# widkyyu/Goal-conditioned-Reinforcement-Learning-with-environmental-and-policy-priors

Measured on AMD Instinct MI355X. Metric: env-steps/sec, higher is better.
Workload: dtype u8

## Files before the change

goal-conditioned-reinforcement-learning-with-environmental-and-policy-priors_amd/_lib.py:

```python
import ctypes as C
import os
import subprocess

_PKG_DIR = os.path.dirname(os.path.abspath(__file__))
LIB_PATH = os.path.join(_PKG_DIR, "libtwoarmy_hip.so")
CSRC_DIR = os.path.join(_PKG_DIR, "csrc")

TW_CELLS = 289
TW_REC_WORDS = 48
TW_DRAW_WORDS = 8
TW_F_AUTORESET = 1
TW_F_POLICY_IDX = 2
TW_F_MATRIX_CODE = 4
TW_F_SLAB_HIPMALLOC = 8

FIELDS = dict(AX=0, AY=1, DIR=2, STEP_COUNT=3, STEP_MOVE=4, PONE=5, PATROL=6, UP1=7, RIGHT2=8, UPD_LONG=9,
              UPD_HORIZ=10, RISK=11, FIRST_ROOM2=12, OBX=13, OBY=16, O1X=19, O1Y=22, O1_VALID=25, O2X=26,
              O2Y=30, O2_VALID=34, GOAL_X=35, GOAL_Y=36, T=37, ERROR=38, MAX_STEPS=39, EPISODES=40,
              LAST_REWARD=41, LAST_TERM=42, LAST_TRUNC=43, WALL_I1=44, WALL_I2=45)

LAUNCH_FIELDS = ("pipelined", "PG", "LAYOUT", "pipe_grid", "E", "FAST", "seq_grid", "T")

ENV_ERRORS = {1: AttributeError, 2: AssertionError, 3: TypeError}

# ... 105 lines not shown
    "mg_nav_path_scan": (C.c_int, [_vp, _i64, _i, _i, _i, _i, _vp, _vp, _vp, _vp, _vp, _vp, _i, _vp, _vp, _vp, _vp, _vp, _vp,
                                   _vp, _vp, _vp]),
    "mg_nav_path_summary_workspace": (C.c_int, [_i, _i]),
    "mg_nav_path_summary": (C.c_int, [_vp, _vp, _vp, _vp, _vp, _vp, _i, _i, _vp, _vp, _vp]),
    "ppo_her_relabel": (C.c_int, [_vp, _vp, _vp, _vp, _vp, _vp, _u64, C.c_uint32, C.c_uint32, _i, _i, _i, _vp, _vp, _vp,
                                  _vp, _vp, _vp, _vp, _vp]),
    "ppo_her_relabel_window": (C.c_int, [_vp, _vp, _vp, _vp, _vp, _vp, _u64, C.c_uint32, C.c_uint32, _i, _i, _i, _i, _vp,
                                         _vp, _vp, _vp, _vp, _vp, _vp, _vp]),
    "ppo_lstm_cell": (C.c_int, [_vp, _vp, C.c_longlong, _vp, _vp, _vp, _i, _i, _vp]),
    "ppo_decoder_frames": (C.c_int, [_vp, _i, _vp, _vp, _vp, _vp, _vp, C.c_float, _vp, _vp]),
    "ppo_gather_stack_u8": (C.c_int, [_vp, _i, _vp, _i, _vp, _vp, _vp, _vp, _vp, _i, _vp, _vp, _vp]),
    "ppo_age_scan": (C.c_int, [_vp, _vp, _vp, _i, _i, _vp, _vp]),
    "ppo_episode_scan": (C.c_int, [_vp, _vp, _vp, _i, _i, _vp, _vp, _vp, _vp, _vp]),
    "ppo_episode_summary": (C.c_int, [_vp, _vp, _vp, _vp, _vp, _vp, _i, _i, _i, C.c_double, C.c_double, _vp, _vp, _vp, _vp,
                                      _vp, _vp]),
    "ppo_episode_summary_workspace": (C.c_int, [_i, _i]),
    "ppo_visit_scan": (C.c_int, [_vp, _vp, _vp, _i, _i, _i, _i, _vp, _vp, _vp, _vp]),
    "ppo_visit_carry_words": (C.c_int, [_i, _i, _i]),
    "ppo_visit_hist": (C.c_int, [_vp, _i, _i, _vp, _vp, _vp, _i, _i, _i, _vp, _vp]),
    "ppo_bonus_table_words": (C.c_int, [_i, _i, _i, _i, _i, _i]),
    "ppo_bonus_workspace_bytes": (_i64, [_i, _i, _i, _i, _i, _i]),
    "ppo_bonus_scan": (C.c_int, [_vp, _vp, _vp, C.c_long, C.c_long, _vp, _vp, _i, _i, _i, _i, _i, _i, _i, C.c_double, _vp, _vp,
                                 _vp, _vp, _vp, _vp, _vp]),
    "ppo_bonus_episode_words": (C.c_int, [_i, _i, _i, _i, _i]),
    "ppo_bonus_scan_episode": (C.c_int, [_vp, _vp, _vp, C.c_long, C.c_long, _vp, _vp, _vp, _vp, _i, _i, _i, _i, _i, _i, _i,
                                         C.c_double, _vp, _vp, _vp, _vp, _vp, _vp]),
    "ppo_bias_relu_nhwc": (C.c_int, [_vp, _vp, _i64, _i, _vp]),
    "ppo_conv1_up4_bias_relu": (C.c_int, [_vp, _i, _i, _vp, _vp, _vp, _vp]),
    "ppo_conv1_up4_bias_relu_c": (C.c_int, [_vp, _i, _i, _i, _vp, _vp, _vp, _vp]),
    "ppo_conv1_up4_bwd_groups": (C.c_int, [_i]),
    "ppo_conv1_up4_bwd": (C.c_int, [_vp, _i, _i, _vp, _vp, _vp, _vp, _vp]),
    "ppo_relu_bwd_bias_grad_nhwc_blocks": (C.c_int, [_i64, _i]),
    "ppo_relu_bwd_bias_grad_nhwc": (C.c_int, [_vp, _vp, _vp, _vp, _i64, _i, _vp]),
})

_lib = None


def exported_symbols():
    return sorted(_SIGS)


def lib():
    global _lib
    if _lib is None:
        if not os.path.exists(LIB_PATH):
            raise TwoarmyLibraryError(
                "%s not built: run `python -c 'import __graft_entry__ as g; g.build()'` "
                "(hipcc --offload-arch=gfx950); there is no CPU fallback" % LIB_PATH)
        import torch
        try:
            h = C.CDLL(LIB_PATH)
        except OSError as ex:
            raise TwoarmyLibraryError("cannot load %s: %s" % (LIB_PATH, ex)) from ex
        for name, (res, args) in _SIGS.items():
            try:
                fn = getattr(h, name)
            except AttributeError as ex:
                raise TwoarmyLibraryError("%s lacks symbol %s" % (LIB_PATH, name)) from ex
            fn.restype, fn.argtypes = res, args
        runtimes = set()
        try:
            with open("/proc/self/maps") as f:
                for line in f:
                    if "libamdhip64" in line:
                        runtimes.add(line.split()[-1])
# ... 17 lines not shown
```

goal-conditioned-reinforcement-learning-with-environmental-and-policy-priors_amd/csrc/ppo_kernels.hip:

```cpp

#include <hip/hip_runtime.h>
#include <float.h>
#include <stdint.h>

#include <type_traits>

#include "launch.h"
#include "philox.h"
#include "twoarmy.h"
#include "twoarmy_ppo.h"

namespace {

constexpr float CAT_EPS = FLT_EPSILON;

template <int A> __device__ __forceinline__ float cat_row(const float *__restrict__ row, float (&p)[A]) {
    float S = 0.f;
#pragma unroll
    for (int k = 0; k < A; ++k) { p[k] = row[k]; S += p[k]; }
    return S;
}
__device__ __forceinline__ float cat_log(float q) { return logf(fminf(fmaxf(q, CAT_EPS), 1.0f - CAT_EPS)); }

template <typename T, int K> __device__ __forceinline__ void block_sum(T (&v)[K], T *lds) {
    const int tid = threadIdx.x;
#pragma unroll
    for (int k = 0; k < K; ++k) lds[k * 256 + tid] = v[k];
    __syncthreads();
    for (int s = 128; s > 0; s >>= 1) {
        if (tid < s) {
#pragma unroll
            for (int k = 0; k < K; ++k) lds[k * 256 + tid] += lds[k * 256 + tid + s];
        }
        __syncthreads();
    }
#pragma unroll
    for (int k = 0; k < K; ++k) v[k] = lds[k * 256];
}

__device__ __forceinline__ float4 relu4(float4 v) {
    return make_float4(fmaxf(v.x, 0.f), fmaxf(v.y, 0.f), fmaxf(v.z, 0.f), fmaxf(v.w, 0.f));
}
__device__ __forceinline__ float4 mask4(float4 g, float4 y) {
    return make_float4(y.x > 0.f ? g.x : 0.f, y.y > 0.f ? g.y : 0.f, y.z > 0.f ? g.z : 0.f, y.w > 0.f ? g.w : 0.f);
}
__device__ __forceinline__ void add4(float4 &acc, const float4 &o) { acc.x += o.x; acc.y += o.y; acc.z += o.z; acc.w += o.w; }
__device__ __forceinline__ float4 fma4(float x, float4 w, float4 acc) {
    return make_float4(fmaf(x, w.x, acc.x), fmaf(x, w.y, acc.y), fmaf(x, w.z, acc.z), fmaf(x, w.w, acc.w));
}

__device__ __forceinline__ float4 slot_sum4(const float4 *red, int rows, int stride, int cq) {
    float4 sum = red[cq];
    for (int r = 1; r < rows; ++r) add4(sum, red[r * stride + cq]);
    return sum;
}

__device__ __forceinline__ uint32_t done_at(const uint8_t *__restrict__ terminated, const uint8_t *__restrict__ truncated,
                                            size_t i) {
    return (uint32_t)(terminated[i] | truncated[i]);
}

template <int A>
__global__ void ppo_sample_kernel(const float *__restrict__ probs, int B, const float *__restrict__ uniforms,
                                  uint32_t k0, uint32_t k1, uint64_t offset, const uint64_t *__restrict__ offset_dev,
                                  int32_t *__restrict__ action, float *__restrict__ logp) {
    const int b = blockIdx.x * blockDim.x + threadIdx.x;
    if (b >= B) return;
    float p[A];
    const float sum = cat_row<A>(probs + (size_t)b * A, p);
    float u;
    if (uniforms) u = uniforms[b];
    else {
        const uint64_t ctr = (uint64_t)b + offset + (offset_dev ? *offset_dev : 0ull);
        uint32_t c0 = (uint32_t)ctr, c1 = (uint32_t)(ctr >> 32), c2 = 0, c3 = 0x54574F53u;
        philox4x32_10(k0, k1, c0, c1, c2, c3);
        u = (float)(c0 >> 8) * (1.0f / 16777216.0f);
    }
    int a = A - 1, last = A - 1;
    float cum = 0.f, qa = 0.f;
    bool found = false;
#pragma unroll
    for (int k = 0; k < A; ++k) {
        const float q = p[k] / sum;
        cum += q;
        if (q > 0.f) last = k;
        if (!found && cum > u) { a = k; found = true; }
    }
    if (!found) a = last;
#pragma unroll
    for (int k = 0; k < A; ++k) if (k == a) qa = p[k] / sum;
    action[b] = a;
    logp[b] = cat_log(qa);
}

__global__ __launch_bounds__(256) void ppo_bias_relu_kernel(float4 *__restrict__ y, const float4 *__restrict__ bias,
                                                            size_t n4, int c4) {
    const size_t stride = (size_t)gridDim.x * blockDim.x;
    for (size_t i = (size_t)blockIdx.x * blockDim.x + threadIdx.x; i < n4; i += stride) {
        float4 v = y[i];
        add4(v, bias[i % c4]);
        y[i] = relu4(v);
    }
}

__global__ __launch_bounds__(256) void ppo_relu_bwd_bias_grad_kernel(const float4 *__restrict__ gy,
                                                                     const float4 *__restrict__ y,
                                                                     float4 *__restrict__ gx,
                                                                     float4 *__restrict__ partial, size_t n_pixels,
                                                                     int c4, int pixels_per_block) {
    __shared__ float4 red[256];
    const int rows = 256 / c4;
    const int cq = threadIdx.x % c4, row = threadIdx.x / c4;
    const size_t p0 = (size_t)blockIdx.x * pixels_per_block;
    const size_t p1 = p0 + pixels_per_block < n_pixels ? p0 + pixels_per_block : n_pixels;
    float4 acc = make_float4(0.f, 0.f, 0.f, 0.f);
    if (row < rows) {
        for (size_t px = p0 + row; px < p1; px += rows) {
            const size_t i = px * c4 + cq;
            const float4 o = mask4(gy[i], y[i]);
            gx[i] = o;
            add4(acc, o);
        }
    }
    red[threadIdx.x] = acc;
    __syncthreads();
    if (row == 0) partial[(size_t)blockIdx.x * c4 + cq] = slot_sum4(red, rows, c4, cq);
}

template <int F> __device__ __forceinline__ void conv1_stage_frame(float *xs, const float *__restrict__ src, int tid) {
    for (int i = tid; i < F * 324; i += 256) {
        const int c = i / 324, r = i - c * 324, y = r / 18, x = r - y * 18;
        xs[i] = (y < 17 && x < 17) ? src[c * 289 + y * 17 + x] : 0.f;
    }
}

template <int F, int CQ>
__global__ __launch_bounds__(256) void ppo_conv1_up4_kernel(const float *__restrict__ frames, const float4 *__restrict__ wf,
                                                            const float4 *__restrict__ bias, float4 *__restrict__ out, int B) {
    __shared__ float xs[F * 18 * 18];
    constexpr int SLOTS = 256 / CQ;
    const int b = blockIdx.x, tid = threadIdx.x;
    const int cq = tid % CQ, slot = tid / CQ;
    conv1_stage_frame<F>(xs, frames + (size_t)b * F * 289, tid);
    __syncthreads();
    const float4 bv = bias[cq];
    float4 *dst = out + (size_t)b * 1089 * CQ;
#pragma unroll 1
    for (int ph = 0; ph < 4; ++ph) {
        const int py = ph >> 1, px = ph & 1;
        float4 w[4 * F];
#pragma unroll
        for (int k = 0; k < 4 * F; ++k) w[k] = wf[(ph * 4 * F + k) * CQ + cq];
        const int ny = 17 - py, nx = 17 - px;
        for (int q = slot; q < ny * nx; q += SLOTS) {
            const int m = q / nx, n = q - m * nx;
            float4 acc = bv;
#pragma unroll
            for (int t = 0; t < 4; ++t) {
                const int ty = t >> 1, tx = t & 1;
#pragma unroll
                for (int c = 0; c < F; ++c) acc = fma4(xs[c * 324 + (m + ty) * 18 + n + tx], w[t * F + c], acc);
            }
            dst[((2 * m + py) * 33 + 2 * n + px) * CQ + cq] = relu4(acc);
        }
    }
}

template <int F>
__global__ __launch_bounds__(256) void ppo_conv1_up4_bwd_kernel(const float *__restrict__ frames, const float4 *__restrict__ gy,
                                                                const float4 *__restrict__ y, float4 *__restrict__ gw_part,
                                                                float4 *__restrict__ gb_part, int B) {
    __shared__ float xs[F * 18 * 18];
    __shared__ float4 red[256];
    const int tid = threadIdx.x, cq = tid & 15, slot = tid >> 4;
    const int ph = blockIdx.y, py = ph >> 1, px = ph & 1;
    const int ny = 17 - py, nx = 17 - px;
    float4 acc[4 * F];
#pragma unroll
    for (int k = 0; k < 4 * F; ++k) acc[k] = make_float4(0.f, 0.f, 0.f, 0.f);
    float4 accb = make_float4(0.f, 0.f, 0.f, 0.f);
    for (int b = blockIdx.x; b < B; b += gridDim.x) {
        __syncthreads();
        conv1_stage_frame<F>(xs, frames + (size_t)b * F * 289, tid);
        __syncthreads();
        const size_t base = (size_t)b * 1089 * 16;
        for (int q = slot; q < ny * nx; q += 16) {
            const int m = q / nx, n = q - m * nx;
            const size_t o = base + (size_t)((2 * m + py) * 33 + 2 * n + px) * 16 + cq;
            const float4 g = mask4(gy[o], y[o]);
            add4(accb, g);
#pragma unroll
            for (int t = 0; t < 4; ++t) {
                const int ty = t >> 1, tx = t & 1;
#pragma unroll
                for (int c = 0; c < F; ++c) acc[t * F + c] = fma4(xs[c * 324 + (m + ty) * 18 + n + tx], g, acc[t * F + c]);
            }
        }
    }
    const size_t wbase = ((size_t)blockIdx.x * 4 + ph) * (4 * F) * 16;
#pragma unroll
    for (int k = 0; k <= 4 * F; ++k) {
        __syncthreads();
        red[tid] = k < 4 * F ? acc[k < 4 * F ? k : 0] : accb;
        __syncthreads();
        if (slot == 0) {
            const float4 sum = slot_sum4(red, 16, 16, cq);
            if (k < 4 * F) gw_part[wbase + (size_t)k * 16 + cq] = sum;
            else gb_part[((size_t)blockIdx.x * 4 + ph) * 16 + cq] = sum;
        }
    }
}

constexpr int GT = 64;

template <int GN>
__global__ __launch_bounds__(256) void ppo_gae_kernel(const float *__restrict__ reward, const float *__restrict__ value,
                                                      const float *__restrict__ next_value,
                                                      const uint8_t *__restrict__ done, float gamma, float lambda,
                                                      int use_done_mask, int T, int N, float *__restrict__ adv,
                                                      float *__restrict__ target, float *__restrict__ ret) {
    __shared__ float sd[GT][GN + 1];
    __shared__ float sc[GT][GN + 1];
// ... 924 lines not shown
int blocks(int64_t n, int per) { return (int)((n + per - 1) / per); }
int blocks_capped(int64_t n, int per, int cap) { return (int)((n + per - 1) / per < cap ? (n + per - 1) / per : cap); }
int ep_summary_blocks(int64_t M) { return blocks_capped(M, EP_BLOCK_ELEMS, EP_MAX_BLOCKS); }
float4 *f4(float *p) { return reinterpret_cast<float4 *>(p); }
const float4 *f4(const float *p) { return reinterpret_cast<const float4 *>(p); }
template <int V> using int_c = std::integral_constant<int, V>;

#define PPO_ACTION_COUNTS(X) X(5) X(2) X(3) X(4) X(7)
bool ppo_actions_ok(int A) {
#define PPO_IS(V) if (A == V) return true;
    PPO_ACTION_COUNTS(PPO_IS)
#undef PPO_IS
    return false;
}
template <typename Fn> void ppo_with_actions(int A, Fn &&fn) {
    switch (A) {
#define PPO_CASE(V) case V: fn(int_c<V>{}); break;
    PPO_ACTION_COUNTS(PPO_CASE)
#undef PPO_CASE
    }
}

template <typename FT>
int gather_stack(const char *what, const FT *frames, int frame_pitch, const float *pos_frames, int N, const int32_t *k_idx,
                 const int32_t *n_idx, const int32_t *age, const float *init_frame, const float *init_pos, int B,
                 float *out, float *pos_out, void *stream) {
    if (!all_set(frames, k_idx, n_idx, age, init_frame, out) || B <= 0 || frame_pitch < TW_CELLS) return TW_E_ARG;
    if (pos_out && !all_set(pos_frames, init_pos)) return TW_E_ARG;
    hipLaunchKernelGGL(ppo_gather_stack_kernel<FT>, dim3(blocks(B, 4)), dim3(256), 0, (hipStream_t)stream, frames, frame_pitch,
                       pos_frames, N, k_idx, n_idx, age, init_frame, init_pos, B, out, pos_out);
    return tw_launched(what);
}

}

extern "C" {

int ppo_sample(const float *probs, int B, int A, const float *uniforms, uint64_t seed, uint64_t offset,
               int32_t *action, float *logp, void *stream) {
    return ppo_sample_dev(probs, B, A, uniforms, seed, offset, nullptr, action, logp, stream);
}

int ppo_sample_dev(const float *probs, int B, int A, const float *uniforms, uint64_t seed, uint64_t offset,
                   const uint64_t *offset_dev, int32_t *action, float *logp, void *stream) {
    if (!all_set(probs, action, logp) || B <= 0 || !ppo_actions_ok(A)) return TW_E_ARG;
    const uint32_t k0 = (uint32_t)seed, k1 = (uint32_t)(seed >> 32);
    ppo_with_actions(A, [&](auto a) {
        hipLaunchKernelGGL(ppo_sample_kernel<decltype(a)::value>, dim3(blocks(B, 256)), dim3(256), 0, (hipStream_t)stream,
                           probs, B, uniforms, k0, k1, offset, offset_dev, action, logp);
    });
    return tw_launched(__func__);
}

int ppo_gae(const float *reward, const float *value, const float *next_value, const uint8_t *done, float gamma,
            float lambda, int use_done_mask, int T, int N, float *adv, float *target, float *ret, void *stream) {
    if (!all_set(reward, value, next_value) || T <= 0 || N <= 0 || (use_done_mask && !done)) return TW_E_ARG;
    auto launch = [&](auto gn) {
        hipLaunchKernelGGL(ppo_gae_kernel<decltype(gn)::value>, dim3(blocks(N, decltype(gn)::value)), dim3(256), 0,
                           (hipStream_t)stream, reward, value, next_value, done, gamma, lambda, use_done_mask, T, N, adv,
                           target, ret);
    };
    if (N >= 16384) launch(int_c<64>{});
    else launch(int_c<16>{});
    return tw_launched(__func__);
}

// ... 167 lines not shown
        !ep_count_ok((int64_t)T * N) || !aligned_natural(reward, carry_return, carry_length, ep_return, ep_length))
        return TW_E_ARG;
    hipLaunchKernelGGL(ppo_episode_scan_kernel, dim3(blocks(N, 64)), dim3(64), 0, (hipStream_t)stream, reward, terminated,
                       truncated, T, N, carry_return, carry_length, ep_return, ep_length);
    return tw_launched(__func__);
}

int ppo_episode_summary_workspace(int T, int N) {
    if (T <= 0 || N <= 0 || !ep_count_ok((int64_t)T * N)) return TW_E_ARG;
    return ep_summary_blocks((int64_t)T * N) * EP_NV;
}

int ppo_episode_summary(const double *ep_return, const int32_t *ep_length, const uint8_t *terminated,
                        const uint8_t *truncated, const float *reward, const int32_t *action, int A, int T, int N,
                        double keep, double gain, double *score, double *summary, int64_t *action_hist,
                        int64_t *reward_hist, double *workspace, void *stream) {
    if (!all_set(ep_return, ep_length, terminated, truncated, reward, summary, reward_hist, workspace) || T <= 0 || N <= 0 ||
        !ppo_actions_ok(A) || !ep_count_ok((int64_t)T * N) ||
        !aligned_natural(ep_return, ep_length, reward, action, score, summary, action_hist, reward_hist, workspace))
        return TW_E_ARG;
    const int64_t M = (int64_t)T * N;
    const int nblocks = ep_summary_blocks(M);
    const int64_t per_block = (M + nblocks - 1) / nblocks;
    const int per_thread = blocks(per_block, 256);
    hipStream_t st = (hipStream_t)stream;
    hipLaunchKernelGGL(ppo_episode_partial_kernel, dim3(nblocks), dim3(256), 0, st, ep_return, ep_length, terminated,
                       truncated, reward, action, M, per_block, per_thread, keep, gain, workspace);
    hipLaunchKernelGGL(ppo_episode_finalize_kernel, dim3(1), dim3(64), 0, st, workspace, nblocks, A, score, summary,
                       action_hist, reward_hist);
    return tw_launched(__func__);
}

int ppo_bias_relu_nhwc(float *y, const float *bias, int64_t n_pixels, int C, void *stream) {
    if (!all_set(y, bias) || n_pixels <= 0 || C <= 0 || (C & 3) || !aligned16(y, bias)) return TW_E_ARG;
    const size_t n4 = (size_t)n_pixels * (C / 4);
    hipLaunchKernelGGL(ppo_bias_relu_kernel, dim3(blocks_capped((int64_t)n4, 256, 8192)), dim3(256), 0, (hipStream_t)stream,
                       f4(y), f4(bias), n4, C / 4);
    return tw_launched(__func__);
}

int ppo_relu_bwd_bias_grad_nhwc_blocks(int64_t n_pixels, int C) {
    if (n_pixels <= 0 || C <= 0 || (C & 3) || C > 256) return TW_E_ARG;
    return blocks_capped(n_pixels, 512, 4096);
}

int ppo_relu_bwd_bias_grad_nhwc(const float *gy, const float *y, float *gx, float *partial, int64_t n_pixels, int C,
                                void *stream) {
    const int nb = ppo_relu_bwd_bias_grad_nhwc_blocks(n_pixels, C);
    if (nb <= 0 || !all_set(gy, y, gx, partial) || !aligned16(gy, y, gx, partial)) return TW_E_ARG;
    const int ppb = blocks(n_pixels, nb);
    hipLaunchKernelGGL(ppo_relu_bwd_bias_grad_kernel, dim3(nb), dim3(256), 0, (hipStream_t)stream, f4(gy), f4(y), f4(gx),
                       f4(partial), (size_t)n_pixels, C / 4, ppb);
    return tw_launched(__func__);
}

int ppo_conv1_up4_bias_relu(const float *frames, int B, int F, const float *folded_w, const float *bias, float *out,
                            void *stream) {
    return ppo_conv1_up4_bias_relu_c(frames, B, F, 64, folded_w, bias, out, stream);
}

int ppo_conv1_up4_bias_relu_c(const float *frames, int B, int F, int C_out, const float *folded_w, const float *bias,
                              float *out, void *stream) {
    if (!all_set(frames, folded_w, bias, out) || B <= 0 || !aligned16(out, folded_w, bias)) return TW_E_ARG;
    auto launch = [&](auto f, auto cq) {
        hipLaunchKernelGGL((ppo_conv1_up4_kernel<decltype(f)::value, decltype(cq)::value>), dim3(B), dim3(256), 0,
                           (hipStream_t)stream, frames, f4(folded_w), f4(bias), f4(out), B);
    };
    if (F == 4 && C_out == 64) launch(int_c<4>{}, int_c<16>{});
    else if (F == 8 && C_out == 64) launch(int_c<8>{}, int_c<16>{});
    else if (F == 1 && C_out == 16) launch(int_c<1>{}, int_c<4>{});
    else return TW_E_ARG;
    return tw_launched(__func__);
}

int ppo_conv1_up4_bwd_groups(int B) { return B <= 0 ? TW_E_ARG : blocks_capped(B, 1, 256); }

int ppo_conv1_up4_bwd(const float *frames, int B, int F, const float *gy, const float *y, float *gw_partial,
                      float *gb_partial, void *stream) {
    const int groups = ppo_conv1_up4_bwd_groups(B);
    if (groups <= 0 || !all_set(frames, gy, y, gw_partial, gb_partial) || !aligned16(gy, y, gw_partial, gb_partial))
        return TW_E_ARG;
    auto launch = [&](auto f) {
        hipLaunchKernelGGL(ppo_conv1_up4_bwd_kernel<decltype(f)::value>, dim3(groups, 4), dim3(256), 0, (hipStream_t)stream,
                           frames, f4(gy), f4(y), f4(gw_partial), f4(gb_partial), B);
    };
    if (F == 4) launch(int_c<4>{});
    else if (F == 8) launch(int_c<8>{});
    else return TW_E_ARG;
    return tw_launched(__func__);
}

int ppo_decoder_frames(const float *z, int n_frames, const float *w1, const float *b1, const float *w2, const float *b2,
                       const float *kfold, float b3, float *frames, void *stream) {
    if (!all_set(z, w1, b1, w2, b2, kfold, frames) || n_frames <= 0) return TW_E_ARG;
    const int grid = blocks_capped(n_frames, 1, 512);
    hipLaunchKernelGGL(ppo_decoder_frames_kernel, dim3(grid), dim3(256), 0, (hipStream_t)stream, z, n_frames, w1, b1, w2,
                       b2, kfold, b3, frames);
    return tw_launched(__func__);
}

int ppo_lstm_cell(const float *gates_a, const float *gates_b, long long ldb, const float *bias, float *c, float *h, int B,
                  int H, void *stream) {
    if ((!gates_a && !gates_b) || !all_set(c, h) || B <= 0 || H <= 0 || (H & 3) || !aligned16(gates_a, gates_b, bias, c, h))
        return TW_E_ARG;
    if (gates_b && ((ldb & 3) || ldb < 4LL * H)) return TW_E_ARG;
    const long long n = (long long)B * (H / 4);
    if (n > 0x7fffffffLL) return TW_E_ARG;
    hipLaunchKernelGGL(ppo_lstm_cell_kernel, dim3(blocks(n, 256)), dim3(256), 0, (hipStream_t)stream, f4(gates_a),
                       f4(gates_b), ldb / 4, f4(bias), f4(c), f4(h), B, H / 4);
    return tw_launched(__func__);
}

}
```

goal-conditioned-reinforcement-learning-with-environmental-and-policy-priors_amd/ppo_ops.py:

```python
import ctypes as C

import torch

from ._marshal import call as _call, constant as _constant, ptr as _p, query as _query

_CL = torch.channels_last


def _pf(t):
    return _p(t.detach().contiguous(), torch.float32)


def _step_outputs(out, want_steps, T, N, dtypes, device):
    if out is None:
        return tuple(torch.empty((T, N), dtype=d, device=device) if want_steps else None for d in dtypes)
    assert out[0].shape == (T, N) and out[1].shape == (T, N)
    return out


def sample(probs, uniforms=None, seed=0, offset=0, offset_dev=None):
    B, A = probs.shape
    action = torch.empty(B, dtype=torch.int32, device=probs.device)
    logp = torch.empty(B, dtype=torch.float32, device=probs.device)
    _call("ppo_sample_dev", probs, _p(probs, torch.float32), B, A, _p(uniforms, torch.float32), seed, offset,
          _p(offset_dev, torch.int64), _p(action), _p(logp))
    return action, logp


def gae(reward, value, next_value, done=None, gamma=0.99, lam=0.0, use_done_mask=False, want_ret=True):
    T, N = reward.shape
    adv = torch.empty_like(reward)
    target = torch.empty_like(reward)
    ret = torch.empty_like(reward) if want_ret else None
# ... 265 lines not shown
                                   lambda kind, N: bonus_episode_words(kind, width, height, n_actions, N))
    _call("ppo_bonus_scan_episode", pos, _p(pos, torch.float32), _p(action, torch.int32), *dirs,
          _p(reward, torch.float32), _p(keep, torch.uint8), _p(terminated, torch.uint8), _p(truncated, torch.uint8), T, N,
          int(width), int(height), int(n_actions), mask, BONUS_FORMS[form], float(scale), _p(state_table, torch.int32),
          _p(action_table, torch.int32), _p(bonus_state, torch.float32), _p(bonus_action, torch.float32),
          _p(reward_out, torch.float32))
    return reward_out


def her_relabel(pos, terminated, truncated, age0, reward, choices=None, seed=0, env_id0=0, step0=0, max_goals=4, skip=0):
    T, N = terminated.shape
    dev = pos.device
    assert pos.shape == (T, N, 2) and pos.is_contiguous() and reward.shape == (T, N)
    if choices is not None:
        assert choices.shape == (T, N, 4) and choices.dtype == torch.int32 and choices.is_contiguous()
    counts = torch.empty(N, dtype=torch.int32, device=dev)
    args = [_p(pos, torch.float32), _p(terminated.contiguous(), torch.uint8), _p(truncated.contiguous(), torch.uint8),
            _p(age0.contiguous(), torch.int32), _p(reward.contiguous(), torch.float32), _p(choices), int(seed),
            int(env_id0), int(step0), T, N, int(max_goals), int(skip)]
    _call("ppo_her_relabel_window", pos, *args, None, _p(counts), None, None, None, None, None)
    incl = torch.cumsum(counts.long(), 0)
    H = int(incl[-1])
    offsets = (incl - counts.long()).contiguous()
    out = dict(t=torch.empty(H, dtype=torch.int32, device=dev), n=torch.empty(H, dtype=torch.int32, device=dev),
               goal=torch.empty((H, 2), dtype=torch.float32, device=dev),
               reward=torch.empty(H, dtype=torch.float32, device=dev), done=torch.empty(H, dtype=torch.uint8, device=dev),
               counts=counts)
    if H:
        _call("ppo_her_relabel_window", pos, *args, _p(offsets), _p(counts), _p(out["t"]), _p(out["n"]), _p(out["goal"]),
              _p(out["reward"]), _p(out["done"]))
    return out


class _ConvBiasReLU(torch.autograd.Function):

    @staticmethod
    def forward(ctx, x, w, b, stride):
        y = torch.ops.aten.convolution(x, w, None, list(stride), [0, 0], [1, 1], False, [0, 0], 1)
        assert y.is_contiguous(memory_format=torch.channels_last), "conv epilogue kernels need channels-last activations"
        B, Cc, H, W = y.shape
        _call("ppo_bias_relu_nhwc", y, _p(y, None, _CL), _pf(b), B * H * W, Cc)
        ctx.save_for_backward(x, w, y)
        ctx.stride = list(stride)
        return y

    @staticmethod
    def backward(ctx, gy):
        x, w, y = ctx.saved_tensors
        gy = gy.contiguous(memory_format=torch.channels_last)
        B, Cc, H, W = y.shape
        npix = B * H * W
        blocks = _query("ppo_relu_bwd_bias_grad_nhwc_blocks", npix, Cc)
        g = torch.empty_like(y)
        partial = torch.empty((blocks, Cc), dtype=torch.float32, device=y.device)
        _call("ppo_relu_bwd_bias_grad_nhwc", y, _p(gy, None, _CL), _p(y, None, _CL), _p(g, None, _CL), _p(partial), npix, Cc)
        gx, gw, _ = torch.ops.aten.convolution_backward(g, x, w, None, ctx.stride, [0, 0], [1, 1], False, [0, 0], 1,
                                                        [bool(ctx.needs_input_grad[0]), True, False])
        return gx, gw, partial.sum(0), None


def conv_bias_relu(x, weight, bias, stride):
    assert x.is_cuda and x.dtype == torch.float32 and x.is_contiguous(memory_format=torch.channels_last)
    return _ConvBiasReLU.apply(x, weight, bias, tuple(stride))


def fold_conv1_weights(w):
    O, F = w.shape[0], w.shape[1]
    w = w.detach().reshape(O, F, 4, 4).float()
    z = torch.zeros_like(w[:, :, 0:1, :])
    rows = torch.stack([torch.cat([w.sum(2, keepdim=True), z], 2),
                        torch.cat([w[:, :, 0:2].sum(2, keepdim=True), w[:, :, 2:4].sum(2, keepdim=True)], 2)], 0)
    zc = torch.zeros_like(rows[..., 0:1])
    cols = torch.stack([torch.cat([rows.sum(-1, keepdim=True), zc], -1),
                        torch.cat([rows[..., 0:2].sum(-1, keepdim=True), rows[..., 2:4].sum(-1, keepdim=True)], -1)], 1)
    return cols.permute(0, 1, 4, 5, 3, 2).contiguous()


@torch.no_grad()
def conv1_up4_bias_relu_infer(frames, weight, bias):
    B, F, _ = frames.shape
    Cout = weight.shape[0]
    y = torch.empty((B, Cout, 33, 33), dtype=torch.float32, device=frames.device, memory_format=torch.channels_last)
    wf = fold_conv1_weights(weight)
    _call("ppo_conv1_up4_bias_relu_c", y, _pf(frames), B, F, Cout, _p(wf), _pf(bias), _p(y, None, _CL))
    return y


class _Conv1Up4(torch.autograd.Function):

    @staticmethod
    def forward(ctx, frames, w, b, wf):
        B, F, _ = frames.shape
        y = torch.empty((B, w.shape[0], 33, 33), dtype=torch.float32, device=frames.device,
                        memory_format=torch.channels_last)
        if wf is None:
            wf = fold_conv1_weights(w)
        fr = frames.contiguous()
        _call("ppo_conv1_up4_bias_relu", y, _p(fr, torch.float32), B, F, _p(wf), _pf(b), _p(y, None, _CL))
        ctx.save_for_backward(fr, w, y)
        return y

    @staticmethod
    def backward(ctx, gy):
        fr, w, y = ctx.saved_tensors
        gy = gy.contiguous(memory_format=torch.channels_last)
        B, F = fr.shape[0], fr.shape[1]
        groups = _query("ppo_conv1_up4_bwd_groups", B)
        gw_part = torch.empty((groups, 2, 2, 2, 2, F, 64), dtype=torch.float32, device=y.device)
        gb_part = torch.empty((groups, 4, 64), dtype=torch.float32, device=y.device)
        _call("ppo_conv1_up4_bwd", y, _p(fr, torch.float32), B, F, _p(gy, None, _CL), _p(y, None, _CL), _p(gw_part),
              _p(gb_part))
        return None, unfold_conv1_grad(gw_part.sum(0)).to(w.dtype), gb_part.sum((0, 1)), None


def unfold_conv1_grad(gwf):
    ty = _constant("conv1_tap_of_row", [[0, 0, 0, 0], [0, 0, 1, 1]], torch.int64, gwf.device)
    out = None
    for py in (0, 1):
        for px in (0, 1):
            g = gwf[py, px][ty[py]][:, ty[px]]
            out = g if out is None else out + g
    return out.permute(3, 2, 0, 1).contiguous()


def conv1_up4_bias_relu(frames, weight, bias, folded=None):
    assert frames.is_cuda and frames.dtype == torch.float32 and weight.shape[2:] == (4, 4) and weight.shape[0] == 64
    return _Conv1Up4.apply(frames, weight, bias, folded)


def fold_decoder_tail(w3):
    m = _constant("decoder_tail_rows", [[0., 0., 1., 1.], [1., 1., 1., 1.], [1., 1., 0., 0.]], w3.dtype, w3.device)
    return torch.einsum("ur,crs,vs->cuv", m, w3[:, 0], m).mul_(1.0 / 16.0).contiguous()


def decoder_frames(z, w1, b1, w2, b2, w3, b3):
    assert z.dim() == 4 and tuple(z.shape[1:]) == (64, 4, 4) and z.dtype == torch.float32
    z = z.contiguous()
    n = z.shape[0]
    out = torch.empty((n, 289), dtype=torch.float32, device=z.device)
    if n:
        _call("ppo_decoder_frames", z, _p(z), n, _pf(w1), _pf(b1), _pf(w2), _pf(b2), _p(fold_decoder_tail(w3.detach())), 0.0,
              _p(out))
        out += b3.detach().view(1, 1)
    return out


def lstm_cell_(gates, c, gates_b=None, bias=None):
    B, H = c.shape
    H4 = 4 * H
    assert c.dtype == torch.float32 and (gates is not None or gates_b is not None)
    assert gates is None or (gates.shape == (B, H4) and gates.dtype == torch.float32)
    pb, ldb = None, 0
    if gates_b is not None:
        assert gates_b.shape == (B, H4) and gates_b.stride(1) == 1 and gates_b.dtype == torch.float32 and gates_b.is_cuda
        pb, ldb = C.c_void_p(gates_b.data_ptr()), gates_b.stride(0) if B > 1 else H4
    h = torch.empty_like(c)
    _call("ppo_lstm_cell", c, _p(gates), pb, ldb, _p(bias), _p(c), _p(h), B, H)
    return h
```

include/twoarmy_ppo.h:

```cpp
#ifndef TWOARMY_PPO_H
#define TWOARMY_PPO_H

#include <stdint.h>

#ifdef __cplusplus
extern "C" {
#endif

int ppo_sample(const float *probs, int B, int A, const float *uniforms, uint64_t seed, uint64_t offset,
               int32_t *action, float *logp, void *stream);
int ppo_sample_dev(const float *probs, int B, int A, const float *uniforms, uint64_t seed, uint64_t offset,
                   const uint64_t *offset_dev, int32_t *action, float *logp, void *stream);

int ppo_gae(const float *reward, const float *value, const float *next_value, const uint8_t *done,
            float gamma, float lambda, int use_done_mask, int T, int N, float *adv, float *target, float *ret,
            void *stream);

int ppo_run_ends(const int32_t *t, const int32_t *n, const float *goal, const uint8_t *done, int64_t H,
                 uint8_t *run_end, int32_t *broken, void *stream);
int ppo_gae_runs(const float *reward, const float *value, const float *next_value, const uint8_t *done,
                 const uint8_t *run_end, float gamma, float lambda, int use_done_mask, int64_t H,
                 float *adv, float *target, float *ret, float *workspace, void *stream);
int ppo_gae_runs_workspace(int64_t H);

// ... 41 lines not shown
int ppo_visit_carry_words(int width, int height, int N);
int ppo_visit_hist(const float *pos, int T, int N, const uint8_t *mask, const int32_t *t_idx, const int32_t *n_idx, int B,
                   int width, int height, int64_t *counts, void *stream);

int ppo_bonus_table_words(int kind, int scope, int width, int height, int n_actions, int N);
int64_t ppo_bonus_workspace_bytes(int kind_mask, int scope, int T, int width, int height, int n_actions);
int ppo_bonus_scan(const float *pos, const int32_t *action, const int32_t *dir, long dir_stride_t, long dir_stride_n,
                   const float *reward, const uint8_t *keep, int T, int N, int width, int height, int n_actions,
                   int kind_mask, int scope, double scale, void *state_table, void *action_table, float *bonus_state,
                   float *bonus_action, float *reward_out, void *workspace, void *stream);

#define BONUS_EPISODE_COUNT_BITS 24
int ppo_bonus_episode_words(int kind, int width, int height, int n_actions, int N);
int ppo_bonus_scan_episode(const float *pos, const int32_t *action, const int32_t *dir, long dir_stride_t, long dir_stride_n,
                           const float *reward, const uint8_t *keep, const uint8_t *terminated, const uint8_t *truncated,
                           int T, int N, int width, int height, int n_actions, int kind_mask, int form, double scale,
                           void *state_table, void *action_table, float *bonus_state, float *bonus_action,
                           float *reward_out, void *stream);

int ppo_her_relabel(const float *pos, const uint8_t *terminated, const uint8_t *truncated, const int32_t *age0,
                    const float *reward, const int32_t *choices, uint64_t seed, uint32_t env_id0, uint32_t step0, int T,
                    int N, int max_goals, const int64_t *offsets, int32_t *counts, int32_t *out_t, int32_t *out_n,
                    float *out_goal, float *out_reward, uint8_t *out_done, void *stream);
int ppo_her_relabel_window(const float *pos, const uint8_t *terminated, const uint8_t *truncated, const int32_t *age0,
                           const float *reward, const int32_t *choices, uint64_t seed, uint32_t env_id0, uint32_t step0,
                           int T, int N, int max_goals, int skip, const int64_t *offsets, int32_t *counts, int32_t *out_t,
                           int32_t *out_n, float *out_goal, float *out_reward, uint8_t *out_done, void *stream);

int ppo_bias_relu_nhwc(float *y, const float *bias, int64_t n_pixels, int C, void *stream);
int ppo_relu_bwd_bias_grad_nhwc_blocks(int64_t n_pixels, int C);
int ppo_relu_bwd_bias_grad_nhwc(const float *gy, const float *y, float *gx, float *partial, int64_t n_pixels, int C,
                                void *stream);

int ppo_conv1_up4_bias_relu(const float *frames, int B, int F, const float *folded_w, const float *bias, float *out,
                            void *stream);
int ppo_conv1_up4_bias_relu_c(const float *frames, int B, int F, int C_out, const float *folded_w, const float *bias,
                              float *out, void *stream);

int ppo_conv1_up4_bwd_groups(int B);
int ppo_conv1_up4_bwd(const float *frames, int B, int F, const float *gy, const float *y, float *gw_partial,
                      float *gb_partial, void *stream);

int ppo_decoder_frames(const float *z, int n_frames, const float *w1, const float *b1, const float *w2, const float *b2,
                       const float *kfold, float b3, float *frames, void *stream);

int ppo_lstm_cell(const float *gates_a, const float *gates_b, long long ldb, const float *bias, float *c, float *h, int B,
                  int H, void *stream);

#ifdef __cplusplus
}
#endif
#endif
```

Measured before the change: 2.994 billion.

## Save ReLU masks as packed bits instead of full activations for backward

Forward conv+bias+ReLU kernels now optionally emit a 1-bit-per-element ReLU mask, built with wave shuffles, and autograd saves that mask instead of the float activation. Backward kernels read the mask words rather than the float tensor. This cuts backward read traffic and saved-tensor memory roughly 32x for these activations, at the cost of extra shuffles and mask writes in forward. It is enabled by default through an environment flag and applies only when grad is enabled and C is a multiple of 64. The metric is env-steps/sec, so the training-side effect may barely register.

```diff
diff --git a/goal-conditioned-reinforcement-learning-with-environmental-and-policy-priors_amd/_lib.py b/goal-conditioned-reinforcement-learning-with-environmental-and-policy-priors_amd/_lib.py
--- a/goal-conditioned-reinforcement-learning-with-environmental-and-policy-priors_amd/_lib.py
+++ b/goal-conditioned-reinforcement-learning-with-environmental-and-policy-priors_amd/_lib.py
@@ -161,6 +161,10 @@
     "ppo_conv1_up4_bwd": (C.c_int, [_vp, _i, _i, _vp, _vp, _vp, _vp, _vp]),
     "ppo_relu_bwd_bias_grad_nhwc_blocks": (C.c_int, [_i64, _i]),
     "ppo_relu_bwd_bias_grad_nhwc": (C.c_int, [_vp, _vp, _vp, _vp, _i64, _i, _vp]),
+    "ppo_bias_relu_bits_nhwc": (C.c_int, [_vp, _vp, _vp, _i64, _i, _vp]),
+    "ppo_relu_bwd_bias_grad_bits_nhwc": (C.c_int, [_vp, _vp, _vp, _vp, _i64, _i, _vp]),
+    "ppo_conv1_up4_bias_relu_bits": (C.c_int, [_vp, _i, _i, _vp, _vp, _vp, _vp, _vp]),
+    "ppo_conv1_up4_bwd_bits": (C.c_int, [_vp, _i, _i, _vp, _vp, _vp, _vp, _vp]),
 })
 
 _lib = None
diff --git a/goal-conditioned-reinforcement-learning-with-environmental-and-policy-priors_amd/csrc/ppo_kernels.hip b/goal-conditioned-reinforcement-learning-with-environmental-and-policy-priors_amd/csrc/ppo_kernels.hip
--- a/goal-conditioned-reinforcement-learning-with-environmental-and-policy-priors_amd/csrc/ppo_kernels.hip
+++ b/goal-conditioned-reinforcement-learning-with-environmental-and-policy-priors_amd/csrc/ppo_kernels.hip
@@ -43,6 +43,21 @@
 }
 __device__ __forceinline__ float4 mask4(float4 g, float4 y) {
     return make_float4(y.x > 0.f ? g.x : 0.f, y.y > 0.f ? g.y : 0.f, y.z > 0.f ? g.z : 0.f, y.w > 0.f ? g.w : 0.f);
+}
+__device__ __forceinline__ uint32_t relu_word(float4 y, int lane) {
+    uint32_t w = ((y.x > 0.f ? 1u : 0u) | (y.y > 0.f ? 2u : 0u) | (y.z > 0.f ? 4u : 0u) | (y.w > 0.f ? 8u : 0u)) << (4 * (lane & 7));
+    w |= (uint32_t)__shfl_xor((int)w, 1);
+    w |= (uint32_t)__shfl_xor((int)w, 2);
+    w |= (uint32_t)__shfl_xor((int)w, 4);
+    return w;
+}
+template <bool BITS> __device__ __forceinline__ float4 relu_bwd4(float4 g, const void *__restrict__ saved, size_t i) {
+    if constexpr (BITS) {
+        const uint32_t m = static_cast<const uint32_t *>(saved)[i >> 3] >> (4 * (i & 7));
+        return make_float4(m & 1u ? g.x : 0.f, m & 2u ? g.y : 0.f, m & 4u ? g.z : 0.f, m & 8u ? g.w : 0.f);
+    } else {
+        return mask4(g, static_cast<const float4 *>(saved)[i]);
+    }
 }
 __device__ __forceinline__ void add4(float4 &acc, const float4 &o) { acc.x += o.x; acc.y += o.y; acc.z += o.z; acc.w += o.w; }
 __device__ __forceinline__ float4 fma4(float x, float4 w, float4 acc) {
@@ -93,18 +108,25 @@
     logp[b] = cat_log(qa);
 }
 
+template <bool BITS>
 __global__ __launch_bounds__(256) void ppo_bias_relu_kernel(float4 *__restrict__ y, const float4 *__restrict__ bias,
-                                                            size_t n4, int c4) {
+                                                            size_t n4, int c4, uint32_t *__restrict__ bits) {
     const size_t stride = (size_t)gridDim.x * blockDim.x;
     for (size_t i = (size_t)blockIdx.x * blockDim.x + threadIdx.x; i < n4; i += stride) {
         float4 v = y[i];
         add4(v, bias[i % c4]);
-        y[i] = relu4(v);
-    }
-}
-
+        v = relu4(v);
+        y[i] = v;
+        if constexpr (BITS) {
+            const uint32_t w = relu_word(v, threadIdx.x);
+            if ((threadIdx.x & 7) == 0) bits[i >> 3] = w;
+        }
+    }
+}
+
+template <bool BITS>
 __global__ __launch_bounds__(256) void ppo_relu_bwd_bias_grad_kernel(const float4 *__restrict__ gy,
-                                                                     const float4 *__restrict__ y,
+                                                                     const void *__restrict__ y,
                                                                      float4 *__restrict__ gx,
                                                                      float4 *__restrict__ partial, size_t n_pixels,
                                                                      int c4, int pixels_per_block) {
@@ -117,7 +139,7 @@
     if (row < rows) {
         for (size_t px = p0 + row; px < p1; px += rows) {
             const size_t i = px * c4 + cq;
-            const float4 o = mask4(gy[i], y[i]);
+            const float4 o = relu_bwd4<BITS>(gy[i], y, i);
             gx[i] = o;
             add4(acc, o);
         }
@@ -134,9 +156,11 @@
     }
 }
 
-template <int F, int CQ>
+template <int F, int CQ, bool BITS>
 __global__ __launch_bounds__(256) void ppo_conv1_up4_kernel(const float *__restrict__ frames, const float4 *__restrict__ wf,
-                                                            const float4 *__restrict__ bias, float4 *__restrict__ out, int B) {
+                                                            const float4 *__restrict__ bias, float4 *__restrict__ out, int B,
+                                                            uint32_t *__restrict__ bits) {
+    static_assert(!BITS || CQ == 16, "mask words are whole for 64 output channels");
     __shared__ float xs[F * 18 * 18];
     constexpr int SLOTS = 256 / CQ;
     const int b = blockIdx.x, tid = threadIdx.x;
@@ -161,14 +185,20 @@
 #pragma unroll
                 for (int c = 0; c < F; ++c) acc = fma4(xs[c * 324 + (m + ty) * 18 + n + tx], w[t * F + c], acc);
             }
-            dst[((2 * m + py) * 33 + 2 * n + px) * CQ + cq] = relu4(acc);
-        }
-    }
-}
-
-template <int F>
+            const int o = ((2 * m + py) * 33 + 2 * n + px) * CQ + cq;
+            const float4 v = relu4(acc);
+            dst[o] = v;
+            if constexpr (BITS) {
+                const uint32_t w = relu_word(v, tid);
+                if ((tid & 7) == 0) bits[((size_t)b * 1089 * CQ + o) >> 3] = w;
+            }
+        }
+    }
+}
+
+template <int F, bool BITS>
 __global__ __launch_bounds__(256) void ppo_conv1_up4_bwd_kernel(const float *__restrict__ frames, const float4 *__restrict__ gy,
-                                                                const float4 *__restrict__ y, float4 *__restrict__ gw_part,
+                                                                const void *__restrict__ y, float4 *__restrict__ gw_part,
                                                                 float4 *__restrict__ gb_part, int B) {
     __shared__ float xs[F * 18 * 18];
     __shared__ float4 red[256];
@@ -187,7 +217,7 @@
         for (int q = slot; q < ny * nx; q += 16) {
             const int m = q / nx, n = q - m * nx;
             const size_t o = base + (size_t)((2 * m + py) * 33 + 2 * n + px) * 16 + cq;
-            const float4 g = mask4(gy[o], y[o]);
+            const float4 g = relu_bwd4<BITS>(gy[o], y, o);
             add4(accb, g);
 #pragma unroll
             for (int t = 0; t < 4; ++t) {
@@ -1178,6 +1208,62 @@
     return tw_launched(what);
 }
 
+bool relu_bits_ok(const uint32_t *mask, int C) { return mask && aligned_natural(mask) && C > 0 && C % 64 == 0; }
+
+int bias_relu(const char *what, float *y, const float *bias, uint32_t *bits, int64_t n_pixels, int C, void *stream) {
+    if (!all_set(y, bias) || n_pixels <= 0 || C <= 0 || (C & 3) || !aligned16(y, bias)) return TW_E_ARG;
+    const size_t n4 = (size_t)n_pixels * (C / 4);
+    auto launch = [&](auto bits_c) {
+        hipLaunchKernelGGL(ppo_bias_relu_kernel<decltype(bits_c)::value != 0>, dim3(blocks_capped((int64_t)n4, 256, 8192)),
+                           dim3(256), 0, (hipStream_t)stream, f4(y), f4(bias), n4, C / 4, bits);
+    };
+    if (bits) launch(int_c<1>{});
+    else launch(int_c<0>{});
+    return tw_launched(what);
+}
+
+template <typename BitsC, typename S>
+int relu_bwd_bias_grad(const char *what, BitsC, const float *gy, const S *saved, float *gx, float *partial, int64_t n_pixels,
+                       int C, void *stream) {
+    const int nb = ppo_relu_bwd_bias_grad_nhwc_blocks(n_pixels, C);
+    if (nb <= 0 || !all_set(gy, saved, gx, partial) || !aligned16(gy, gx, partial)) return TW_E_ARG;
+    const int ppb = blocks(n_pixels, nb);
+    hipLaunchKernelGGL(ppo_relu_bwd_bias_grad_kernel<BitsC::value != 0>, dim3(nb), dim3(256), 0, (hipStream_t)stream, f4(gy),
+                       (const void *)saved, f4(gx), f4(partial), (size_t)n_pixels, C / 4, ppb);
+    return tw_launched(what);
+}
+
+int conv1_up4(const char *what, const float *frames, int B, int F, int C_out, const float *folded_w, const float *bias,
+              float *out, uint32_t *bits, void *stream) {
+    if (!all_set(frames, folded_w, bias, out) || B <= 0 || !aligned16(out, folded_w, bias)) return TW_E_ARG;
+    auto launch = [&](auto f, auto cq, auto bits_c) {
+        hipLaunchKernelGGL((ppo_conv1_up4_kernel<decltype(f)::value, decltype(cq)::value, decltype(bits_c)::value != 0>),
+                           dim3(B), dim3(256), 0, (hipStream_t)stream, frames, f4(folded_w), f4(bias), f4(out), B, bits);
+    };
+    auto either = [&](auto f, auto cq) { if (bits) launch(f, cq, int_c<1>{}); else launch(f, cq, int_c<0>{}); };
+    if (F == 4 && C_out == 64) either(int_c<4>{}, int_c<16>{});
+    else if (F == 8 && C_out == 64) either(int_c<8>{}, int_c<16>{});
+    else if (F == 1 && C_out == 16 && !bits) launch(int_c<1>{}, int_c<4>{}, int_c<0>{});
+    else return TW_E_ARG;
+    return tw_launched(what);
+}
+
+template <typename BitsC, typename S>
+int conv1_up4_bwd(const char *what, BitsC, const float *frames, int B, int F, const float *gy, const S *saved,
+                  float *gw_partial, float *gb_partial, void *stream) {
+    const int groups = ppo_conv1_up4_bwd_groups(B);
+    if (groups <= 0 || !all_set(frames, gy, saved, gw_partial, gb_partial) || !aligned16(gy, gw_partial, gb_partial))
+        return TW_E_ARG;
+    auto launch = [&](auto f) {
+        hipLaunchKernelGGL((ppo_conv1_up4_bwd_kernel<decltype(f)::value, BitsC::value != 0>), dim3(groups, 4), dim3(256), 0,
+                           (hipStream_t)stream, frames, f4(gy), (const void *)saved, f4(gw_partial), f4(gb_partial), B);
+    };
+    if (F == 4) launch(int_c<4>{});
+    else if (F == 8) launch(int_c<8>{});
+    else return TW_E_ARG;
+    return tw_launched(what);
+}
+
 }
 
 extern "C" {
@@ -1411,11 +1497,13 @@
 }
 
 int ppo_bias_relu_nhwc(float *y, const float *bias, int64_t n_pixels, int C, void *stream) {
-    if (!all_set(y, bias) || n_pixels <= 0 || C <= 0 || (C & 3) || !aligned16(y, bias)) return TW_E_ARG;
-    const size_t n4 = (size_t)n_pixels * (C / 4);
-    hipLaunchKernelGGL(ppo_bias_relu_kernel, dim3(blocks_capped((int64_t)n4, 256, 8192)), dim3(256), 0, (hipStream_t)stream,
-                       f4(y), f4(bias), n4, C / 4);
-    return tw_launched(__func__);
+    return bias_relu(__func__, y, bias, nullptr, n_pixels, C, stream);
+}
+
+int ppo_bias_relu_bits_nhwc(float *y, const float *bias, uint32_t *mask, int64_t n_pixels, int C,
+                            struct ihipStream_t *stream) {
+    if (!relu_bits_ok(mask, C)) return TW_E_ARG;
+    return bias_relu(__func__, y, bias, mask, n_pixels, C, stream);
 }
 
 int ppo_relu_bwd_bias_grad_nhwc_blocks(int64_t n_pixels, int C) {
@@ -1425,12 +1513,14 @@
 
 int ppo_relu_bwd_bias_grad_nhwc(const float *gy, const float *y, float *gx, float *partial, int64_t n_pixels, int C,
                                 void *stream) {
-    const int nb = ppo_relu_bwd_bias_grad_nhwc_blocks(n_pixels, C);
-    if (nb <= 0 || !all_set(gy, y, gx, partial) || !aligned16(gy, y, gx, partial)) return TW_E_ARG;
-    const int ppb = blocks(n_pixels, nb);
-    hipLaunchKernelGGL(ppo_relu_bwd_bias_grad_kernel, dim3(nb), dim3(256), 0, (hipStream_t)stream, f4(gy), f4(y), f4(gx),
-                       f4(partial), (size_t)n_pixels, C / 4, ppb);
-    return tw_launched(__func__);
+    if (!aligned16(y)) return TW_E_ARG;
+    return relu_bwd_bias_grad(__func__, int_c<0>{}, gy, y, gx, partial, n_pixels, C, stream);
+}
+
+int ppo_relu_bwd_bias_grad_bits_nhwc(const float *gy, const uint32_t *mask, float *gx, float *partial, int64_t n_pixels,
+                                     int C, struct ihipStream_t *stream) {
+    if (!relu_bits_ok(mask, C)) return TW_E_ARG;
+    return relu_bwd_bias_grad(__func__, int_c<1>{}, gy, mask, gx, partial, n_pixels, C, stream);
 }
 
 int ppo_conv1_up4_bias_relu(const float *frames, int B, int F, const float *folded_w, const float *bias, float *out,
@@ -1440,33 +1530,27 @@
 
 int ppo_conv1_up4_bias_relu_c(const float *frames, int B, int F, int C_out, const float *folded_w, const float *bias,
                               float *out, void *stream) {
-    if (!all_set(frames, folded_w, bias, out) || B <= 0 || !aligned16(out, folded_w, bias)) return TW_E_ARG;
-    auto launch = [&](auto f, auto cq) {
-        hipLaunchKernelGGL((ppo_conv1_up4_kernel<decltype(f)::value, decltype(cq)::value>), dim3(B), dim3(256), 0,
-                           (hipStream_t)stream, frames, f4(folded_w), f4(bias), f4(out), B);
-    };
-    if (F == 4 && C_out == 64) launch(int_c<4>{}, int_c<16>{});
-    else if (F == 8 && C_out == 64) launch(int_c<8>{}, int_c<16>{});
-    else if (F == 1 && C_out == 16) launch(int_c<1>{}, int_c<4>{});
-    else return TW_E_ARG;
-    return tw_launched(__func__);
+    return conv1_up4(__func__, frames, B, F, C_out, folded_w, bias, out, nullptr, stream);
+}
+
+int ppo_conv1_up4_bias_relu_bits(const float *frames, int B, int F, const float *folded_w, const float *bias, float *out,
+                                 uint32_t *mask, struct ihipStream_t *stream) {
+    if (!relu_bits_ok(mask, 64)) return TW_E_ARG;
+    return conv1_up4(__func__, frames, B, F, 64, folded_w, bias, out, mask, stream);
 }
 
 int ppo_conv1_up4_bwd_groups(int B) { return B <= 0 ? TW_E_ARG : blocks_capped(B, 1, 256); }
 
 int ppo_conv1_up4_bwd(const float *frames, int B, int F, const float *gy, const float *y, float *gw_partial,
                       float *gb_partial, void *stream) {
-    const int groups = ppo_conv1_up4_bwd_groups(B);
-    if (groups <= 0 || !all_set(frames, gy, y, gw_partial, gb_partial) || !aligned16(gy, y, gw_partial, gb_partial))
-        return TW_E_ARG;
-    auto launch = [&](auto f) {
-        hipLaunchKernelGGL(ppo_conv1_up4_bwd_kernel<decltype(f)::value>, dim3(groups, 4), dim3(256), 0, (hipStream_t)stream,
-                           frames, f4(gy), f4(y), f4(gw_partial), f4(gb_partial), B);
-    };
-    if (F == 4) launch(int_c<4>{});
-    else if (F == 8) launch(int_c<8>{});
-    else return TW_E_ARG;
-    return tw_launched(__func__);
+    if (!aligned16(y)) return TW_E_ARG;
+    return conv1_up4_bwd(__func__, int_c<0>{}, frames, B, F, gy, y, gw_partial, gb_partial, stream);
+}
+
+int ppo_conv1_up4_bwd_bits(const float *frames, int B, int F, const float *gy, const uint32_t *mask, float *gw_partial,
+                           float *gb_partial, struct ihipStream_t *stream) {
+    if (!relu_bits_ok(mask, 64)) return TW_E_ARG;
+    return conv1_up4_bwd(__func__, int_c<1>{}, frames, B, F, gy, mask, gw_partial, gb_partial, stream);
 }
 
 int ppo_decoder_frames(const float *z, int n_frames, const float *w1, const float *b1, const float *w2, const float *b2,
diff --git a/goal-conditioned-reinforcement-learning-with-environmental-and-policy-priors_amd/ppo_ops.py b/goal-conditioned-reinforcement-learning-with-environmental-and-policy-priors_amd/ppo_ops.py
--- a/goal-conditioned-reinforcement-learning-with-environmental-and-policy-priors_amd/ppo_ops.py
+++ b/goal-conditioned-reinforcement-learning-with-environmental-and-policy-priors_amd/ppo_ops.py
@@ -1,4 +1,5 @@
 import ctypes as C
+import os
 
 import torch
 
@@ -330,36 +331,63 @@
     return out
 
 
+RELU_BITS = os.environ.get("TWOARMY_RELU_BITS", "1") != "0"
+
+
+def _wants_bits(C):
+    return RELU_BITS and torch.is_grad_enabled() and C % 64 == 0
+
+
+def relu_mask_like(y):
+    assert y.numel() % 32 == 0
+    return torch.empty(y.numel() // 32, dtype=torch.int32, device=y.device)
+
+
+def pack_relu_mask(y):
+    flat = (y.detach().permute(0, 2, 3, 1).reshape(-1, 32) > 0).to(torch.int64)
+    words = (flat << torch.arange(32, device=y.device)).sum(1)
+    return torch.where(words >= 2 ** 31, words - 2 ** 32, words).to(torch.int32)
+
+
 class _ConvBiasReLU(torch.autograd.Function):
 
     @staticmethod
-    def forward(ctx, x, w, b, stride):
+    def forward(ctx, x, w, b, stride, bits):
         y = torch.ops.aten.convolution(x, w, None, list(stride), [0, 0], [1, 1], False, [0, 0], 1)
         assert y.is_contiguous(memory_format=torch.channels_last), "conv epilogue kernels need channels-last activations"
         B, Cc, H, W = y.shape
-        _call("ppo_bias_relu_nhwc", y, _p(y, None, _CL), _pf(b), B * H * W, Cc)
-        ctx.save_for_backward(x, w, y)
-        ctx.stride = list(stride)
+        ctx.stride, ctx.shape = list(stride), y.shape
+        if bits and any(ctx.needs_input_grad):
+            mask = relu_mask_like(y)
+            _call("ppo_bias_relu_bits_nhwc", y, _p(y, None, _CL), _pf(b), _p(mask), B * H * W, Cc)
+            ctx.save_for_backward(x, w, mask)
+        else:
+            _call("ppo_bias_relu_nhwc", y, _p(y, None, _CL), _pf(b), B * H * W, Cc)
+            ctx.save_for_backward(x, w, y)
         return y
 
     @staticmethod
     def backward(ctx, gy):
-        x, w, y = ctx.saved_tensors
+        x, w, saved = ctx.saved_tensors
         gy = gy.contiguous(memory_format=torch.channels_last)
-        B, Cc, H, W = y.shape
+        B, Cc, H, W = ctx.shape
         npix = B * H * W
         blocks = _query("ppo_relu_bwd_bias_grad_nhwc_blocks", npix, Cc)
-        g = torch.empty_like(y)
-        partial = torch.empty((blocks, Cc), dtype=torch.float32, device=y.device)
-        _call("ppo_relu_bwd_bias_grad_nhwc", y, _p(gy, None, _CL), _p(y, None, _CL), _p(g, None, _CL), _p(partial), npix, Cc)
+        g = torch.empty(ctx.shape, dtype=torch.float32, device=gy.device, memory_format=_CL)
+        partial = torch.empty((blocks, Cc), dtype=torch.float32, device=gy.device)
+        if saved.dtype == torch.int32:
+            _call("ppo_relu_bwd_bias_grad_bits_nhwc", gy, _p(gy, None, _CL), _p(saved), _p(g, None, _CL), _p(partial), npix, Cc)
+        else:
+            _call("ppo_relu_bwd_bias_grad_nhwc", gy, _p(gy, None, _CL), _p(saved, None, _CL), _p(g, None, _CL), _p(partial),
+                  npix, Cc)
         gx, gw, _ = torch.ops.aten.convolution_backward(g, x, w, None, ctx.stride, [0, 0], [1, 1], False, [0, 0], 1,
                                                         [bool(ctx.needs_input_grad[0]), True, False])
-        return gx, gw, partial.sum(0), None
+        return gx, gw, partial.sum(0), None, None
 
 
 def conv_bias_relu(x, weight, bias, stride):
     assert x.is_cuda and x.dtype == torch.float32 and x.is_contiguous(memory_format=torch.channels_last)
-    return _ConvBiasReLU.apply(x, weight, bias, tuple(stride))
+    return _ConvBiasReLU.apply(x, weight, bias, tuple(stride), _wants_bits(weight.shape[0]))
 
 
 def fold_conv1_weights(w):
@@ -387,28 +415,34 @@
 class _Conv1Up4(torch.autograd.Function):
 
     @staticmethod
-    def forward(ctx, frames, w, b, wf):
+    def forward(ctx, frames, w, b, wf, bits):
         B, F, _ = frames.shape
         y = torch.empty((B, w.shape[0], 33, 33), dtype=torch.float32, device=frames.device,
                         memory_format=torch.channels_last)
         if wf is None:
             wf = fold_conv1_weights(w)
         fr = frames.contiguous()
-        _call("ppo_conv1_up4_bias_relu", y, _p(fr, torch.float32), B, F, _p(wf), _pf(b), _p(y, None, _CL))
-        ctx.save_for_backward(fr, w, y)
+        if bits and any(ctx.needs_input_grad):
+            mask = relu_mask_like(y)
+            _call("ppo_conv1_up4_bias_relu_bits", y, _p(fr, torch.float32), B, F, _p(wf), _pf(b), _p(y, None, _CL), _p(mask))
+            ctx.save_for_backward(fr, w, mask)
+        else:
+            _call("ppo_conv1_up4_bias_relu", y, _p(fr, torch.float32), B, F, _p(wf), _pf(b), _p(y, None, _CL))
+            ctx.save_for_backward(fr, w, y)
         return y
 
     @staticmethod
     def backward(ctx, gy):
-        fr, w, y = ctx.saved_tensors
+        fr, w, saved = ctx.saved_tensors
         gy = gy.contiguous(memory_format=torch.channels_last)
         B, F = fr.shape[0], fr.shape[1]
         groups = _query("ppo_conv1_up4_bwd_groups", B)
-        gw_part = torch.empty((groups, 2, 2, 2, 2, F, 64), dtype=torch.float32, device=y.device)
-        gb_part = torch.empty((groups, 4, 64), dtype=torch.float32, device=y.device)
-        _call("ppo_conv1_up4_bwd", y, _p(fr, torch.float32), B, F, _p(gy, None, _CL), _p(y, None, _CL), _p(gw_part),
-              _p(gb_part))
-        return None, unfold_conv1_grad(gw_part.sum(0)).to(w.dtype), gb_part.sum((0, 1)), None
+        gw_part = torch.empty((groups, 2, 2, 2, 2, F, 64), dtype=torch.float32, device=gy.device)
+        gb_part = torch.empty((groups, 4, 64), dtype=torch.float32, device=gy.device)
+        bits = saved.dtype == torch.int32
+        _call("ppo_conv1_up4_bwd_bits" if bits else "ppo_conv1_up4_bwd", gy, _p(fr, torch.float32), B, F, _p(gy, None, _CL),
+              _p(saved) if bits else _p(saved, None, _CL), _p(gw_part), _p(gb_part))
+        return None, unfold_conv1_grad(gw_part.sum(0)).to(w.dtype), gb_part.sum((0, 1)), None, None
 
 
 def unfold_conv1_grad(gwf):
@@ -423,7 +457,7 @@
 
 def conv1_up4_bias_relu(frames, weight, bias, folded=None):
     assert frames.is_cuda and frames.dtype == torch.float32 and weight.shape[2:] == (4, 4) and weight.shape[0] == 64
-    return _Conv1Up4.apply(frames, weight, bias, folded)
+    return _Conv1Up4.apply(frames, weight, bias, folded, _wants_bits(weight.shape[0]))
 
 
 def fold_decoder_tail(w3):
diff --git a/include/twoarmy_ppo.h b/include/twoarmy_ppo.h
--- a/include/twoarmy_ppo.h
+++ b/include/twoarmy_ppo.h
@@ -97,6 +97,12 @@
 int ppo_relu_bwd_bias_grad_nhwc(const float *gy, const float *y, float *gx, float *partial, int64_t n_pixels, int C,
                                 void *stream);
 
+struct ihipStream_t;
+int ppo_bias_relu_bits_nhwc(float *y, const float *bias, uint32_t *mask, int64_t n_pixels, int C,
+                            struct ihipStream_t *stream);
+int ppo_relu_bwd_bias_grad_bits_nhwc(const float *gy, const uint32_t *mask, float *gx, float *partial, int64_t n_pixels,
+                                     int C, struct ihipStream_t *stream);
+
 int ppo_conv1_up4_bias_relu(const float *frames, int B, int F, const float *folded_w, const float *bias, float *out,
                             void *stream);
 int ppo_conv1_up4_bias_relu_c(const float *frames, int B, int F, int C_out, const float *folded_w, const float *bias,
@@ -105,6 +111,11 @@
 int ppo_conv1_up4_bwd_groups(int B);
 int ppo_conv1_up4_bwd(const float *frames, int B, int F, const float *gy, const float *y, float *gw_partial,
                       float *gb_partial, void *stream);
+
+int ppo_conv1_up4_bias_relu_bits(const float *frames, int B, int F, const float *folded_w, const float *bias, float *out,
+                                 uint32_t *mask, struct ihipStream_t *stream);
+int ppo_conv1_up4_bwd_bits(const float *frames, int B, int F, const float *gy, const uint32_t *mask, float *gw_partial,
+                           float *gb_partial, struct ihipStream_t *stream);
 
 int ppo_decoder_frames(const float *z, int n_frames, const float *w1, const float *b1, const float *w2, const float *b2,
                        const float *kfold, float b3, float *frames, void *stream);
```

Result: no change. 2.987 billion (median of 2 runs) (-0.2%).
